# borglab/gtsfm

Measured on NVIDIA H100. Metric: image_pairs_per_sec, higher is better.
Workload: dtype f32

## Files before the change

gtsfm_b200/csrc/gemm_ws.cuh:

```cuda
#pragma once
#include "tma.cuh"

constexpr int GW_MAXP = 16;
constexpr int GW_M = 128, GW_N = 128, GW_K = 64;
constexpr int GW_A_BYTES = GW_M * GW_K * 2;
constexpr int GW_B_BYTES = GW_N * GW_K * 2;
constexpr int GW_STAGE_BYTES = 2 * GW_A_BYTES + 2 * GW_B_BYTES;
constexpr int GW_STAGES = 2;
constexpr int GW_PITCH = GW_N + 8;
constexpr int GW_STG_BYTES = GW_M * GW_PITCH * 4;
constexpr int GW_RB = 8;
constexpr int GW_EW = 4;
constexpr int GW_THREADS = 512;
constexpr size_t GW_SMEM = GW_STAGES * GW_STAGE_BYTES + GW_STG_BYTES + 1024  + 256 ;
constexpr int GW_SEGS = 3;

struct GemmProblem {
  const float* resid;
  float* C;
  __half *Ch[GW_SEGS], *Cl[GW_SEGS];
  const float *cs, *sn;
  int M, N, ldc;
  int vec4;
  int tiles_n;
  int tile_end;
};
struct GemmWsMaps {
  CUtensorMap a1h[GW_MAXP], a1l[GW_MAXP];
  CUtensorMap a2h[GW_MAXP], a2l[GW_MAXP];
  CUtensorMap bh[GW_MAXP], bl[GW_MAXP];
};
struct GemmWsArgs {
  GemmProblem p[GW_MAXP];
  int nprob, tiles;
  int K1, K2;
  int b_per_problem;
  const float* bias;
  int ldr;
  float scale;
  int ldch;
  int head_major;
  int relu;
  int gelu;
  int lo_unscaled;
  int seg_n;
  int rot_mask;
  int* err_flag;
};

static __device__ __noinline__ float gelu_erf(float x) { return 0.5f * x * (1.0f + erff(x * 0.70710678118654752440f)); }

static __global__ void __launch_bounds__(GW_THREADS, 1) k_gemm_ws(const __grid_constant__ GemmWsMaps maps, const __grid_constant__ GemmWsArgs g) {
  extern __shared__ unsigned char gw_raw[];
  const uint32_t raw = tc::smem_u32(gw_raw);
  const uint32_t smem0 = (raw + 1023u) & ~1023u;
  unsigned char* sm = gw_raw + (smem0 - raw);
  float* stg = reinterpret_cast<float*>(sm + GW_STAGES * GW_STAGE_BYTES);
  uint64_t* full = reinterpret_cast<uint64_t*>(sm + GW_STAGES * GW_STAGE_BYTES + GW_STG_BYTES);
  uint64_t* empty = full + GW_STAGES;
  uint64_t* sfull = empty + GW_STAGES;
  uint64_t* sempty = sfull + 1;

  const int t = threadIdx.x, warp = t >> 5, lane = t & 31;
  const int nk = (g.K1 + g.K2) / GW_K;

  if (t == 0) {
    for (int s = 0; s < GW_STAGES; ++s) tc::mbar_init(&full[s], 1), tc::mbar_init(&empty[s], 8);
    tc::mbar_init(sfull, 256);
    tc::mbar_init(sempty, 32 * GW_EW);
    tc::fence_mbar_init();
    tc::tma_prefetch_desc(&maps.bh[0]);
    tc::tma_prefetch_desc(&maps.bl[0]);
  }
  __syncthreads();
  bool ok = true;

  auto decode = [&](int tile, int& z, int& m0, int& n0) {
    z = 0;
    while (z + 1 < g.nprob && tile >= g.p[z].tile_end) ++z;
    const int local = tile - (z ? g.p[z - 1].tile_end : 0);
    const int mt = local / g.p[z].tiles_n;
    n0 = (local - mt * g.p[z].tiles_n) * GW_N;
    m0 = mt * GW_M;
  };

  if (warp >= 12) {
    asm volatile("setmaxnreg.dec.sync.aligned.u32 40;\n" ::: "memory");
    if (warp == 12 && lane == 0) {
      int gk = 0;
      for (int tile = blockIdx.x; tile < g.tiles; tile += gridDim.x) {
        int z, m0, n0;
        decode(tile, z, m0, n0);
        const int zb = g.b_per_problem ? z : 0;
        for (int kc = 0; kc < nk; ++kc, ++gk) {
          const int s = gk % GW_STAGES;
          if (gk >= GW_STAGES) ok = tc::mbar_wait(&empty[s], ((gk / GW_STAGES) - 1) & 1) && ok;
          const int k0 = kc * GW_K;
          const bool seg2 = k0 >= g.K1;
          const CUtensorMap* ah = seg2 ? &maps.a2h[z] : &maps.a1h[z];
          const CUtensorMap* al = seg2 ? &maps.a2l[z] : &maps.a1l[z];
          const int ka = seg2 ? k0 - g.K1 : k0;
          const uint32_t sA = smem0 + s * GW_STAGE_BYTES, sB = sA + 2 * GW_A_BYTES;
          tc::mbar_expect_tx(&full[s], GW_STAGE_BYTES);
          tc::tma_load_2d(sA, ah, &full[s], ka, m0);
          tc::tma_load_2d(sA + GW_A_BYTES, al, &full[s], ka, m0);
          tc::tma_load_2d(sB, &maps.bh[zb], &full[s], k0, n0);
          tc::tma_load_2d(sB + GW_B_BYTES, &maps.bl[zb], &full[s], k0, n0);
        }
      }
    }
  } else if (warp < 8) {
    asm volatile("setmaxnreg.inc.sync.aligned.u32 184;\n" ::: "memory");
    const int wg = warp >> 2;
    const int r0 = wg * 64 + (warp & 3) * 16 + (lane >> 2);
    const int c2 = (lane & 3) * 2;
    int gk = 0, it = 0;
    for (int tile = blockIdx.x; tile < g.tiles; tile += gridDim.x, ++it) {
      float acc0[64], acc1[64];
      for (int kc = 0; kc < nk; ++kc, ++gk) {
        const int s = gk % GW_STAGES;
        ok = tc::mbar_wait(&full[s], (gk / GW_STAGES) & 1) && ok;
        const uint32_t aH = smem0 + s * GW_STAGE_BYTES + wg * (64 * 128), aL = aH + GW_A_BYTES;
        const uint32_t bH = smem0 + s * GW_STAGE_BYTES + 2 * GW_A_BYTES, bL = bH + GW_B_BYTES;
        const uint64_t dAh = tc::wg_desc_sw128(aH), dAl = tc::wg_desc_sw128(aL), dBh = tc::wg_desc_sw128(bH), dBl = tc::wg_desc_sw128(bL);
        tc::wg_fence();
#pragma unroll
        for (int ks = 0; ks < GW_K / 16; ++ks) {
          const uint64_t adv = (uint64_t)(ks * 2);
          const uint32_t first = (kc == 0 && ks == 0) ? 0u : 1u;
          tc::wg_ss_n128(acc0, dAh + adv, dBh + adv, first);
          tc::wg_ss_n128(acc1, dAh + adv, dBl + adv, first);
          tc::wg_ss_n128(acc1, dAl + adv, dBh + adv, 1u);
        }
        tc::wg_commit();
        if (kc > 0) {
          tc::wg_wait<1>();
          if (lane == 0) tc::mbar_arrive(&empty[(gk - 1) % GW_STAGES]);
        }
      }
      tc::wg_wait<0>();
      if (lane == 0) tc::mbar_arrive(&empty[(gk - 1) % GW_STAGES]);

      if (it > 0) ok = tc::mbar_wait(sempty, (it - 1) & 1) && ok;
#pragma unroll
      for (int j = 0; j < 16; ++j)
#pragma unroll
        for (int h = 0; h < 2; ++h) {
          const int i = 4 * j + 2 * h;
          *reinterpret_cast<float2*>(stg + (r0 + 8 * h) * GW_PITCH + 8 * j + c2) =
              make_float2(fmaf(acc1[i], tc::LO_INV, acc0[i]), fmaf(acc1[i + 1], tc::LO_INV, acc0[i + 1]));
        }
      tc::mbar_arrive(sfull);
    }
  } else {
    asm volatile("setmaxnreg.dec.sync.aligned.u32 104;\n" ::: "memory");
    const int ew = warp - 8;
    const int c = 4 * lane;
    const float scale = g.scale;
    const int relu = g.relu, gelu = g.gelu, hm = g.head_major, lo_unscaled = g.lo_unscaled, ldr = g.ldr, ldch = g.ldch;
    int it = 0;
    for (int tile = blockIdx.x; tile < g.tiles; tile += gridDim.x, ++it) {
      int z, m0, n0;
      decode(tile, z, m0, n0);
      const GemmProblem& pb = g.p[z];
      const float* resid = pb.resid;
      float* C = pb.C;
      const int sg = g.seg_n ? n0 / g.seg_n : 0;
      __half *Ch = pb.Ch[sg], *Cl = pb.Cl[sg];
      const bool rot = (g.rot_mask >> sg) & 1;
      const int M = pb.M, ldc = pb.ldc;
      const int n = n0 + c;
      const int ncols = min(4, pb.N - n);
      const bool vec = pb.vec4 && ncols == 4;
      const int rows = min(GW_M, M - m0);
      float b4[4] = {0.f, 0.f, 0.f, 0.f};
      if (g.bias)
#pragma unroll
        for (int e = 0; e < 4; ++e)
          if (e < ncols) b4[e] = __ldg(g.bias + n + e);
      const int ns = n - sg * g.seg_n;
      const size_t hm_col = (size_t)(ns >> 6) * M * 64 + (ns & 63);
      const bool vres = resid && vec;
      const int rp = (ns & 63) >> 1;
      float4 rr[GW_RB];
      auto load_rows = [&](int rb) {
        if (rot) {
#pragma unroll
          for (int i = 0; i < GW_RB; ++i)
            if (rb + GW_EW * i < rows) {
              const size_t o = (size_t)(m0 + rb + GW_EW * i) * 32 + rp;
              const float2 cc = __ldg(reinterpret_cast<const float2*>(pb.cs + o)), ss = __ldg(reinterpret_cast<const float2*>(pb.sn + o));
              rr[i] = make_float4(cc.x, cc.y, ss.x, ss.y);
            }
        } else {
#pragma unroll
          for (int i = 0; i < GW_RB; ++i)
            if (rb + GW_EW * i < rows) rr[i] = *reinterpret_cast<const float4*>(resid + (size_t)(m0 + rb + GW_EW * i) * ldr + n);
        }
      };
      if (vres || rot) load_rows(ew);
      ok = tc::mbar_wait(sfull, it & 1) && ok;
      auto pre = [&](int r, float* v) {
        const float4 a = *reinterpret_cast<const float4*>(stg + r * GW_PITCH + c);
        v[0] = a.x, v[1] = a.y, v[2] = a.z, v[3] = a.w;
#pragma unroll
        for (int e = 0; e < 4; ++e) {
          v[e] = (v[e] + b4[e]) * scale;
          if (relu) v[e] = fmaxf(v[e], 0.f);
          if (gelu) v[e] = gelu_erf(v[e]);
        }
      };
      if (ncols > 0 && vec) {
        for (int rb = ew; rb < rows; rb += GW_EW * GW_RB) {
          if ((vres || rot) && rb != ew) load_rows(rb);
#pragma unroll
          for (int i = 0; i < GW_RB; ++i) {
            const int r = rb + GW_EW * i;
            if (r >= rows) break;
            const int row = m0 + r;
            float v[4];
            pre(r, v);
            if (resid) v[0] += rr[i].x, v[1] += rr[i].y, v[2] += rr[i].z, v[3] += rr[i].w;
            if (rot) {
              const float c0 = rr[i].x, c1 = rr[i].y, s0 = rr[i].z, s1 = rr[i].w;
              const float a0 = __fadd_rn(__fmul_rn(v[0], c0), __fmul_rn(-v[1], s0)), a1 = __fadd_rn(__fmul_rn(v[1], c0), __fmul_rn(v[0], s0));
              const float a2 = __fadd_rn(__fmul_rn(v[2], c1), __fmul_rn(-v[3], s1)), a3 = __fadd_rn(__fmul_rn(v[3], c1), __fmul_rn(v[2], s1));
              v[0] = a0, v[1] = a1, v[2] = a2, v[3] = a3;
            }
            const size_t off = hm ? hm_col + (size_t)row * 64 : (size_t)row * ldc + n;
            if (C) *reinterpret_cast<float4*>(C + off) = make_float4(v[0], v[1], v[2], v[3]);
            if (Ch) {
              const size_t off_s = hm ? off : (size_t)row * ldch + n;
              uint32_t h01, l01, h23, l23;
              if (lo_unscaled) {
                tc::split2_unscaled_clamped(v[0], v[1], h01, l01);
                tc::split2_unscaled_clamped(v[2], v[3], h23, l23);
              } else {
                tc::split2(v[0], v[1], h01, l01);
                tc::split2(v[2], v[3], h23, l23);
              }
              *reinterpret_cast<uint2*>(Ch + off_s) = make_uint2(h01, h23);
              *reinterpret_cast<uint2*>(Cl + off_s) = make_uint2(l01, l23);
            }
          }
        }
      } else if (ncols > 0) {
#pragma unroll 1
        for (int r = ew; r < rows; r += GW_EW) {
          const int row = m0 + r;
          float v[4];
          pre(r, v);
          const size_t off_c = hm ? hm_col + (size_t)row * 64 : (size_t)row * ldc + n;
          const size_t off_s = hm ? hm_col + (size_t)row * 64 : (size_t)row * ldch + n;
#pragma unroll
          for (int e = 0; e < 4; ++e) {
            if (e >= ncols) break;
            if (resid) v[e] += resid[(size_t)row * ldr + n + e];
            if (C) C[off_c + e] = v[e];
            if (Ch) {
              __half hh, ll;
              if (lo_unscaled) tc::split_h_unscaled(v[e], hh, ll);
              else tc::split_h(v[e], hh, ll);
              Ch[off_s + e] = hh;
              Cl[off_s + e] = ll;
            }
          }
        }
      }
      tc::mbar_arrive(sempty);
    }
  }
  if (!ok && g.err_flag) *g.err_flag = 1;
}
```

gtsfm_b200/csrc/linear.cuh:

```cuda
#pragma once
#include "attn_ps.cuh"
#include "common.cuh"
#include "gemm.cuh"
#include "gemm_ws.cuh"

struct TcWeights {
  const float* f;
  const __half* h;
  const __half* l;
  int* err;
  bool use_tc;
  DevBuf* attn_part = nullptr;
  DevBuf* attn_ml = nullptr;
  DevBuf* attn_cnt = nullptr;
  int sm_count = 132;
};

struct Pl {
  __half* hi;
  __half* lo;
};
static inline Pl planes_of(const DevBuf& b, size_t elems) { return {b.as<__half>(), b.as<__half>() + elems}; }

struct LinArgs {
  const float* a1f = nullptr;
  Pl a1p{nullptr, nullptr};
  int lda1 = 0, K1 = 0;
  const float* a2f = nullptr;
  Pl a2p{nullptr, nullptr};
  int lda2 = 0, K2 = 0;
  const float* w = nullptr;
  const float* bf = nullptr;
  Pl bp{nullptr, nullptr};
  int ldb = 0;
  const float* bias = nullptr;
  float scale = 1.f;
  const float* resid = nullptr;
  int ldr = 0;
  float* cf = nullptr;
  int ldc = 0;
  Pl cp{nullptr, nullptr};
  int ldch = 0;
  int head_major = 0;
  bool tc_want_f32 = false;
  int relu = 0;
  int gelu = 0;
  int lo_unscaled = 0;
  int M = 0, N = 0;
  int seg_n = 0;
  float* seg_f[GW_SEGS] = {};
  Pl seg_p[GW_SEGS] = {};
  int rot_mask = 0;
  const float *cs = nullptr, *sn = nullptr;
};

static int run_linear(b2_context* ctx, cudaStream_t st, const TcWeights& tw, const LinArgs* a, int np, const char* site = nullptr) {
  if (np <= 0) return B2_OK;
  if (np > GW_MAXP) return b2_fail(ctx, B2_ERR_ARG, "run_linear: too many problems in one launch");
  const LinArgs& a0 = a[0];
  const int nseg = a0.seg_n > 0 ? a0.N / a0.seg_n : 1;
  if (a0.seg_n > 0 && (a0.seg_n % GW_N || a0.N != nseg * a0.seg_n || nseg > GW_SEGS || !a0.head_major || a0.resid || a0.tc_want_f32 ||
                       (a0.rot_mask && (!a0.cs || !a0.sn))))
    return b2_fail(ctx, B2_ERR_ARG, "run_linear: column segments need N = seg_n x (<= 3), seg_n % 128 == 0, head-major planes, "
                                    "no residual or fp32 output, and a rotary table when rotary is on");
  if (!tw.use_tc) {
    if (a0.rot_mask) return b2_fail(ctx, B2_ERR_ARG, "run_linear: the rotary epilogue exists on the wgmma path only");
    for (int i = 0; i < np; ++i) {
      const LinArgs& x = a[i];
      if (x.M <= 0 || x.N <= 0) continue;
      if (x.gelu) return b2_fail(ctx, B2_ERR_ARG, "run_linear: the GELU epilogue exists on the wgmma path only");
      if (x.K1 % GB_K || x.K2 % GB_K || x.lda1 % 4 || x.lda2 % 4 || x.ldb % 4)
        return b2_fail(ctx, B2_ERR_ARG, "run_linear: the SIMT GEMM needs K1, K2 multiples of 16 and lda1, lda2, ldb multiples of 4");
    }
    for (int i = 0; i < np; ++i) {
      const LinArgs& x = a[i];
      if (x.M <= 0 || x.N <= 0) continue;
      for (int s = 0; s < nseg; ++s) {
        const int c0 = s * x.seg_n;
        GemmArgs g{};
        g.A1 = x.a1f, g.lda1 = x.lda1, g.K1 = x.K1, g.A2 = x.a2f, g.lda2 = x.lda2, g.K2 = x.K2;
        g.B = (x.w ? x.w : x.bf) + (size_t)c0 * x.ldb, g.ldb = x.ldb, g.C = x.seg_n ? x.seg_f[s] : x.cf, g.ldc = x.ldc, g.M = x.M;
        g.N = x.seg_n ? x.seg_n : x.N;
        g.bias = x.bias ? x.bias + c0 : nullptr, g.resid = x.resid, g.ldr = x.ldr, g.scale = x.scale, g.head_major = x.head_major;
        g.relu = x.relu;
        int rc = launch_gemm(ctx, st, g);
        if (rc) return rc;
      }
    }
    return B2_OK;
  }
  if (a0.K1 % GW_K || a0.K2 % GW_K) return b2_fail(ctx, B2_ERR_ARG, "run_linear: the wgmma GEMM needs K1 and K2 multiples of 64");
  if (!tma_encoder()) return b2_fail(ctx, B2_ERR_CUDA, "cuTensorMapEncodeTiled is not available (driver too old?)");
  const bool per_b = a0.w == nullptr;
  static thread_local GemmWsMaps maps;
  GemmWsArgs q{};
  double work = 0.0;
  bool ok = true;
  int nz = 0, tiles = 0;
  for (int i = 0; i < np; ++i) {
    const LinArgs& x = a[i];
    if (x.M <= 0 || x.N <= 0) continue;
    ok = ok && tma_map_2d(&maps.a1h[nz], x.a1p.hi, x.M, x.K1, x.lda1, GW_M) && tma_map_2d(&maps.a1l[nz], x.a1p.lo, x.M, x.K1, x.lda1, GW_M);
    if (x.K2 > 0)
      ok = ok && tma_map_2d(&maps.a2h[nz], x.a2p.hi, x.M, x.K2, x.lda2, GW_M) && tma_map_2d(&maps.a2l[nz], x.a2p.lo, x.M, x.K2, x.lda2, GW_M);
    if (per_b || nz == 0) {
      const __half *bh, *bl;
      if (x.w) {
        const size_t off = (size_t)(x.w - tw.f);
        bh = tw.h + off, bl = tw.l + off;
      } else {
        bh = x.bp.hi, bl = x.bp.lo;
      }
      ok = ok && tma_map_2d(&maps.bh[nz], bh, x.N, x.K1 + x.K2, x.ldb, GW_N) && tma_map_2d(&maps.bl[nz], bl, x.N, x.K1 + x.K2, x.ldb, GW_N);
    }
    GemmProblem& pr = q.p[nz];
    pr.resid = x.resid, pr.C = x.tc_want_f32 ? x.cf : nullptr, pr.M = x.M, pr.N = x.N, pr.ldc = x.ldc;
    for (int s = 0; s < GW_SEGS; ++s) {
      const Pl p = x.seg_n ? (s < nseg ? x.seg_p[s] : Pl{nullptr, nullptr}) : (s == 0 ? x.cp : Pl{nullptr, nullptr});
      pr.Ch[s] = p.hi, pr.Cl[s] = p.lo;
    }
    pr.cs = x.cs, pr.sn = x.sn;
    {
      auto al16 = [](const void* q) { return (reinterpret_cast<uintptr_t>(q) & 15) == 0; };
      auto al8 = [](const void* q) { return (reinterpret_cast<uintptr_t>(q) & 7) == 0; };
      const bool hm = x.head_major != 0;
      bool v = al16(pr.resid) && (x.ldr % 4 == 0 || !pr.resid) && al16(pr.C) && (hm || x.ldc % 4 == 0 || !pr.C);
      v = v && (hm || x.ldch % 4 == 0 || !pr.Ch[0]);
      for (int s = 0; s < GW_SEGS; ++s) v = v && al8(pr.Ch[s]) && al8(pr.Cl[s]);
      v = v && al8(pr.cs) && al8(pr.sn);
      pr.vec4 = v ? 1 : 0;
      if (x.seg_n && !v) return b2_fail(ctx, B2_ERR_ARG, "run_linear: column segments need 8-byte aligned planes and rotary tables");
    }
    pr.tiles_n = cdiv(x.N, GW_N);
    tiles += cdiv(x.M, GW_M) * pr.tiles_n;
    pr.tile_end = tiles;
    work += 2.0 * x.M * x.N * (x.K1 + x.K2);
    ++nz;
  }
  if (nz == 0) return B2_OK;
  if (!ok) return b2_fail(ctx, B2_ERR_CUDA, "cuTensorMapEncodeTiled failed");
  q.nprob = nz, q.tiles = tiles, q.K1 = a0.K1, q.K2 = a0.K2, q.b_per_problem = per_b ? 1 : 0;
  q.bias = a0.bias, q.ldr = a0.ldr, q.scale = a0.scale, q.ldch = a0.ldch;
  q.head_major = a0.head_major, q.relu = a0.relu, q.gelu = a0.gelu, q.lo_unscaled = a0.lo_unscaled, q.err_flag = tw.err;
  q.seg_n = a0.seg_n, q.rot_mask = a0.rot_mask;
  const std::string name = site ? std::string("k_gemm_ws/") + site : std::string("k_gemm_ws");
  b2_prof_work(ctx, name.c_str(), work);
  B2_LAUNCH_NAMED(ctx, name.c_str(), k_gemm_ws, tiles < tw.sm_count ? tiles : tw.sm_count, GW_THREADS, GW_SMEM, st, maps, q);
  B2_CHECK_LAUNCH(ctx);
  return B2_OK;
}

struct FlashPlanes {
  Pl q, k, v, o;
  int nq, nk;
  int heads, ldo;
};
static int run_flash_planes(b2_context* ctx, cudaStream_t st, const TcWeights& tw, const FlashPlanes* jobs, int np, float scale,
                            bool fp16_single = false) {
  if (np <= 0) return B2_OK;
  if (np > AP_MAXP) return b2_fail(ctx, B2_ERR_ARG, "run_flash: too many problems in one launch");
  if (!tma_encoder() || !tw.attn_part) return b2_fail(ctx, B2_ERR_CUDA, "wgmma attention needs cuTensorMapEncodeTiled and its scratch buffers");
  static thread_local AttnPsMaps tmaps;
  AttnPsArgs pa{};
  bool okm = true;
  int items = 0, nz = 0, W = 0, tmax = 0;
  double work = 0.0;
  for (int i = 0; i < np; ++i) {
    const FlashPlanes& j = jobs[i];
    if (j.nq <= 0 || j.nk <= 0) continue;
    AttnPsProblem& p = pa.p[nz];
    p.Qh = j.q.hi, p.Ql = j.q.lo, p.Oh = j.o.hi, p.Ol = j.o.lo, p.Nq = j.nq, p.Nk = j.nk, p.ldo = j.ldo;
    p.qt = cdiv(j.nq, 2 * AW_Q), p.tiles = cdiv(j.nk, AW_KV);
    p.item0 = items;
    items += p.qt * j.heads;
    W += p.qt * j.heads * p.tiles;
    p.w_end = W;
    tmax = p.tiles > tmax ? p.tiles : tmax;
    const uint64_t rows = (uint64_t)j.heads * j.nk;
    okm = okm && tma_map_2d(&tmaps.kh[nz], j.k.hi, rows, 64, 64, AW_KV) && tma_map_2d(&tmaps.kl[nz], j.k.lo, rows, 64, 64, AW_KV);
    okm = okm && tma_map_2d(&tmaps.vh[nz], j.v.hi, rows, 64, 64, AW_KV) && tma_map_2d(&tmaps.vl[nz], j.v.lo, rows, 64, 64, AW_KV);
    work += j.heads * 2.0 * 2.0 * 64 * (double)j.nq * j.nk;
    ++nz;
  }
  if (nz == 0) return B2_OK;
  if (!okm) return b2_fail(ctx, B2_ERR_CUDA, "cuTensorMapEncodeTiled failed (attention)");
  pa.nprob = nz, pa.W = W;
  int ncta = W < tw.sm_count ? W : tw.sm_count;
  pa.quota = cdiv(W, ncta);
  ncta = cdiv(W, pa.quota);
  pa.max_splits = cdiv(tmax, pa.quota) + 1;
  B2_CUDA(ctx, tw.attn_part->ensure((size_t)items * pa.max_splits * 256 * 64 * 4));
  B2_CUDA(ctx, tw.attn_ml->ensure((size_t)items * pa.max_splits * 256 * 2 * 4));
  {
    DevBuf& cnt = *tw.attn_cnt;
    const size_t need = (size_t)items * 2 * sizeof(int);
    if (cnt.cap < need) {
      B2_CUDA(ctx, cnt.ensure(need * 4));
      B2_CUDA(ctx, cudaMemsetAsync(cnt.p, 0, cnt.cap, st));
    }
    pa.arrivals = cnt.as<int>();
  }
  pa.Opart = tw.attn_part->as<float>(), pa.ml = tw.attn_ml->as<float>();
  pa.scale = scale, pa.err_flag = tw.err;
  b2_prof_work(ctx, "k_flash_ps", work);
  if (fp16_single) B2_LAUNCH(ctx, k_flash_ps<true>, ncta, AS_THREADS, AS_SMEM, st, tmaps, pa);
  else B2_LAUNCH(ctx, k_flash_ps<false>, ncta, AS_THREADS, AS_SMEM, st, tmaps, pa);
  B2_CHECK_LAUNCH(ctx);
  return B2_OK;
}

struct FlashJob {
  const DevBuf *q, *k, *v, *o;
  int nq, nk;
  int capq, capk;
};
static int run_flash(b2_context* ctx, cudaStream_t st, const TcWeights& tw, const FlashJob* jobs, int np, float scale, bool fp16_single = false) {
  if (np <= 0) return B2_OK;
  if (np > AP_MAXP) return b2_fail(ctx, B2_ERR_ARG, "run_flash: too many problems in one launch");
  if (!tw.use_tc) {
    for (int i = 0; i < np; ++i) {
      const FlashJob& j = jobs[i];
      int rc = launch_flash(ctx, st, j.q->as<float>(), j.k->as<float>(), j.v->as<float>(), j.o->as<float>(), j.nq, j.nk, scale);
      if (rc) return rc;
    }
    return B2_OK;
  }
  FlashPlanes fp[AP_MAXP];
  for (int i = 0; i < np; ++i) {
    const FlashJob& j = jobs[i];
    fp[i] = {planes_of(*j.q, (size_t)j.capq * 256), planes_of(*j.k, (size_t)j.capk * 256), planes_of(*j.v, (size_t)j.capk * 256),
             planes_of(*j.o, (size_t)j.capq * 256), j.nq, j.nk, 4, 256};
  }
  return run_flash_planes(ctx, st, tw, fp, np, scale, fp16_single);
}
```

gtsfm_b200/csrc/tma.cuh:

```cuda
#pragma once
#include <cuda.h>
#include <cuda_fp16.h>

#include "common.cuh"
#include "tc.cuh"

namespace tc {
__device__ __forceinline__ void mbar_expect_tx(uint64_t* bar, uint32_t bytes) {
  asm volatile("mbarrier.arrive.expect_tx.shared::cta.b64 _, [%0], %1;" ::"r"(smem_u32(bar)), "r"(bytes) : "memory");
}
__device__ __forceinline__ void tma_load_2d(uint32_t dst_smem, const CUtensorMap* map, uint64_t* bar, int x, int y) {
  asm volatile(
      "cp.async.bulk.tensor.2d.shared::cluster.global.tile.mbarrier::complete_tx::bytes [%0], [%1, {%3, %4}], [%2];"
      ::"r"(dst_smem), "l"(reinterpret_cast<uint64_t>(map)), "r"(smem_u32(bar)), "r"(x), "r"(y)
      : "memory");
}
__device__ __forceinline__ void tma_prefetch_desc(const CUtensorMap* map) {
  asm volatile("prefetch.tensormap [%0];" ::"l"(reinterpret_cast<uint64_t>(map)) : "memory");
}
}

typedef CUresult (*PFN_encodeTiled)(CUtensorMap*, CUtensorMapDataType, cuuint32_t, void*, const cuuint64_t*, const cuuint64_t*,
                                    const cuuint32_t*, const cuuint32_t*, CUtensorMapInterleave, CUtensorMapSwizzle,
                                    CUtensorMapL2promotion, CUtensorMapFloatOOBfill);

static inline PFN_encodeTiled tma_encoder() {
  static PFN_encodeTiled fn = nullptr;
  if (!fn) {
    void* p = nullptr;
    cudaDriverEntryPointQueryResult q;
    if (cudaGetDriverEntryPoint("cuTensorMapEncodeTiled", &p, cudaEnableDefault, &q) == cudaSuccess && q == cudaDriverEntryPointSuccess)
      fn = reinterpret_cast<PFN_encodeTiled>(p);
  }
  return fn;
}

static inline bool tma_map_2d(CUtensorMap* out, const __half* base, uint64_t rows, uint64_t cols, uint64_t ld, uint32_t box_rows) {
  PFN_encodeTiled enc = tma_encoder();
  if (!enc || !base) return false;
  cuuint64_t dims[2] = {cols, rows};
  cuuint64_t strides[1] = {ld * sizeof(__half)};
  cuuint32_t box[2] = {64, box_rows};
  cuuint32_t estr[2] = {1, 1};
  return enc(out, CU_TENSOR_MAP_DATA_TYPE_FLOAT16, 2, const_cast<__half*>(base), dims, strides, box, estr, CU_TENSOR_MAP_INTERLEAVE_NONE,
             CU_TENSOR_MAP_SWIZZLE_128B, CU_TENSOR_MAP_L2_PROMOTION_L2_256B, CU_TENSOR_MAP_FLOAT_OOB_FILL_NONE) == CUDA_SUCCESS;
}

static __global__ void k_split_f32(const float* __restrict__ x, size_t n, __half* __restrict__ hi, __half* __restrict__ lo) {
  size_t i = (size_t)blockIdx.x * blockDim.x + threadIdx.x;
  if (i >= n) return;
  __half h, l;
  tc::split_h(x[i], h, l);
  hi[i] = h;
  lo[i] = l;
}
```

Baseline: 130.9.

## Route GEMM epilogue stores through swizzled smem and TMA bulk tensor stores

Result: faster. 132.5 (median of 6 runs) (+1.2%).

```diff
diff --git a/gtsfm_b200/csrc/gemm_ws.cuh b/gtsfm_b200/csrc/gemm_ws.cuh
--- a/gtsfm_b200/csrc/gemm_ws.cuh
+++ b/gtsfm_b200/csrc/gemm_ws.cuh
@@ -7,8 +7,8 @@
 constexpr int GW_B_BYTES = GW_N * GW_K * 2;
 constexpr int GW_STAGE_BYTES = 2 * GW_A_BYTES + 2 * GW_B_BYTES;
 constexpr int GW_STAGES = 2;
-constexpr int GW_PITCH = GW_N + 8;
-constexpr int GW_STG_BYTES = GW_M * GW_PITCH * 4;
+constexpr int GW_BLK = GW_M * 128;
+constexpr int GW_STG_BYTES = 4 * GW_BLK;
 constexpr int GW_RB = 8;
 constexpr int GW_EW = 4;
 constexpr int GW_THREADS = 512;
@@ -29,6 +29,8 @@
   CUtensorMap a1h[GW_MAXP], a1l[GW_MAXP];
   CUtensorMap a2h[GW_MAXP], a2l[GW_MAXP];
   CUtensorMap bh[GW_MAXP], bl[GW_MAXP];
+  CUtensorMap c[GW_MAXP];
+  CUtensorMap ch[GW_MAXP][GW_SEGS], cl[GW_MAXP][GW_SEGS];
 };
 struct GemmWsArgs {
   GemmProblem p[GW_MAXP];
@@ -67,7 +69,7 @@
   if (t == 0) {
     for (int s = 0; s < GW_STAGES; ++s) tc::mbar_init(&full[s], 1), tc::mbar_init(&empty[s], 8);
     tc::mbar_init(sfull, 256);
-    tc::mbar_init(sempty, 32 * GW_EW);
+    tc::mbar_init(sempty, 1);
     tc::fence_mbar_init();
     tc::tma_prefetch_desc(&maps.bh[0]);
     tc::tma_prefetch_desc(&maps.bl[0]);
@@ -147,7 +149,8 @@
 #pragma unroll
         for (int h = 0; h < 2; ++h) {
           const int i = 4 * j + 2 * h;
-          *reinterpret_cast<float2*>(stg + (r0 + 8 * h) * GW_PITCH + 8 * j + c2) =
+          const int off = (j >> 2) * GW_BLK + (r0 + 8 * h) * 128 + (((2 * (j & 3) + (c2 >> 2)) ^ (lane >> 2)) << 4) + (c2 & 3) * 4;
+          *reinterpret_cast<float2*>(reinterpret_cast<unsigned char*>(stg) + off) =
               make_float2(fmaf(acc1[i], tc::LO_INV, acc0[i]), fmaf(acc1[i + 1], tc::LO_INV, acc0[i + 1]));
         }
       tc::mbar_arrive(sfull);
@@ -156,8 +159,14 @@
     asm volatile("setmaxnreg.dec.sync.aligned.u32 104;\n" ::: "memory");
     const int ew = warp - 8;
     const int c = 4 * lane;
+    const bool leader = t == 256;
     const float scale = g.scale;
     const int relu = g.relu, gelu = g.gelu, hm = g.head_major, lo_unscaled = g.lo_unscaled, ldr = g.ldr, ldch = g.ldch;
+    unsigned char* stgb = reinterpret_cast<unsigned char*>(stg);
+    const uint32_t stg_s = tc::smem_u32(stg);
+    const int o32_0 = (lane >> 3) * GW_BLK + (((lane & 7) ^ ew) << 4), o32_1 = o32_0 ^ (4 << 4);
+    const int oh_0 = 2 * (lane >> 4) * GW_BLK + ((((lane & 15) >> 1) ^ ew) << 4) + (lane & 1) * 8, oh_1 = oh_0 ^ (4 << 4);
+    auto epi_sync = [] { asm volatile("bar.sync 1, 128;" ::: "memory"); };
     int it = 0;
     for (int tile = blockIdx.x; tile < g.tiles; tile += gridDim.x, ++it) {
       int z, m0, n0;
@@ -168,10 +177,10 @@
       const int sg = g.seg_n ? n0 / g.seg_n : 0;
       __half *Ch = pb.Ch[sg], *Cl = pb.Cl[sg];
       const bool rot = (g.rot_mask >> sg) & 1;
-      const int M = pb.M, ldc = pb.ldc;
+      const int M = pb.M, N = pb.N, ldc = pb.ldc;
       const int n = n0 + c;
-      const int ncols = min(4, pb.N - n);
-      const bool vec = pb.vec4 && ncols == 4;
+      const int ncols = min(4, N - n);
+      const bool fast = pb.vec4 != 0;
       const int rows = min(GW_M, M - m0);
       float b4[4] = {0.f, 0.f, 0.f, 0.f};
       if (g.bias)
@@ -179,8 +188,7 @@
         for (int e = 0; e < 4; ++e)
           if (e < ncols) b4[e] = __ldg(g.bias + n + e);
       const int ns = n - sg * g.seg_n;
-      const size_t hm_col = (size_t)(ns >> 6) * M * 64 + (ns & 63);
-      const bool vres = resid && vec;
+      const bool vres = resid && fast && ncols > 0;
       const int rp = (ns & 63) >> 1;
       float4 rr[GW_RB];
       auto load_rows = [&](int rb) {
@@ -200,9 +208,8 @@
       };
       if (vres || rot) load_rows(ew);
       ok = tc::mbar_wait(sfull, it & 1) && ok;
-      auto pre = [&](int r, float* v) {
-        const float4 a = *reinterpret_cast<const float4*>(stg + r * GW_PITCH + c);
-        v[0] = a.x, v[1] = a.y, v[2] = a.z, v[3] = a.w;
+      auto ld_row = [&](int r, int p) { return *reinterpret_cast<const float4*>(stgb + r * 128 + (p ? o32_1 : o32_0)); };
+      auto fin = [&](float* v) {
 #pragma unroll
         for (int e = 0; e < 4; ++e) {
           v[e] = (v[e] + b4[e]) * scale;
@@ -210,46 +217,113 @@
           if (gelu) v[e] = gelu_erf(v[e]);
         }
       };
-      if (ncols > 0 && vec) {
-        for (int rb = ew; rb < rows; rb += GW_EW * GW_RB) {
-          if ((vres || rot) && rb != ew) load_rows(rb);
-#pragma unroll
-          for (int i = 0; i < GW_RB; ++i) {
-            const int r = rb + GW_EW * i;
-            if (r >= rows) break;
-            const int row = m0 + r;
-            float v[4];
-            pre(r, v);
-            if (resid) v[0] += rr[i].x, v[1] += rr[i].y, v[2] += rr[i].z, v[3] += rr[i].w;
-            if (rot) {
-              const float c0 = rr[i].x, c1 = rr[i].y, s0 = rr[i].z, s1 = rr[i].w;
-              const float a0 = __fadd_rn(__fmul_rn(v[0], c0), __fmul_rn(-v[1], s0)), a1 = __fadd_rn(__fmul_rn(v[1], c0), __fmul_rn(v[0], s0));
-              const float a2 = __fadd_rn(__fmul_rn(v[2], c1), __fmul_rn(-v[3], s1)), a3 = __fadd_rn(__fmul_rn(v[3], c1), __fmul_rn(v[2], s1));
-              v[0] = a0, v[1] = a1, v[2] = a2, v[3] = a3;
-            }
-            const size_t off = hm ? hm_col + (size_t)row * 64 : (size_t)row * ldc + n;
-            if (C) *reinterpret_cast<float4*>(C + off) = make_float4(v[0], v[1], v[2], v[3]);
-            if (Ch) {
-              const size_t off_s = hm ? off : (size_t)row * ldch + n;
-              uint32_t h01, l01, h23, l23;
-              if (lo_unscaled) {
-                tc::split2_unscaled_clamped(v[0], v[1], h01, l01);
-                tc::split2_unscaled_clamped(v[2], v[3], h23, l23);
-              } else {
-                tc::split2(v[0], v[1], h01, l01);
-                tc::split2(v[2], v[3], h23, l23);
+      auto put_planes = [&](int r, int p, const float* v, bool sync = true) {
+        uint32_t h01, l01, h23, l23;
+        if (lo_unscaled) {
+          tc::split2_unscaled_clamped(v[0], v[1], h01, l01);
+          tc::split2_unscaled_clamped(v[2], v[3], h23, l23);
+        } else {
+          tc::split2(v[0], v[1], h01, l01);
+          tc::split2(v[2], v[3], h23, l23);
+        }
+        unsigned char* q = stgb + r * 128 + (p ? oh_1 : oh_0);
+        if (sync) __syncwarp();
+        *reinterpret_cast<uint2*>(q) = make_uint2(h01, h23);
+        *reinterpret_cast<uint2*>(q + GW_BLK) = make_uint2(l01, l23);
+      };
+      auto store_half = [&](int hf, bool f32) {
+        const int y = m0 + 64 * hf;
+        const uint32_t src = stg_s + hf * 64 * 128;
+        if (f32) {
+#pragma unroll 1
+          for (int b = 0; b < 4; ++b) {
+            const int col = n0 + 32 * b;
+            if (col < N) tc::tma_store_3d(&maps.c[z], src + b * GW_BLK, hm ? (col & 63) : col, y, hm ? col >> 6 : 0);
+          }
+        } else {
+#pragma unroll 1
+          for (int k = 0; k < 2; ++k) {
+            const int col = n0 + 64 * k;
+            if (col >= N) break;
+            const int x = hm ? 0 : col, h = hm ? (col - sg * g.seg_n) >> 6 : 0;
+            tc::tma_store_3d(&maps.ch[z][sg], src + 2 * k * GW_BLK, x, y, h);
+            tc::tma_store_3d(&maps.cl[z][sg], src + (2 * k + 1) * GW_BLK, x, y, h);
+          }
+        }
+        tc::bulk_commit();
+      };
+      if (fast) {
+        const bool direct_planes = Ch && !C;
+        for (int hf = 0; hf < 2 && 64 * hf < rows; ++hf) {
+          for (int rb = 64 * hf + ew; rb < 64 * (hf + 1) && rb < rows; rb += GW_EW * GW_RB) {
+            if ((vres || rot) && rb != ew) load_rows(rb);
+            auto post = [&](int i, float* v) {
+              if (vres) v[0] += rr[i].x, v[1] += rr[i].y, v[2] += rr[i].z, v[3] += rr[i].w;
+              if (rot) {
+                const float c0 = rr[i].x, c1 = rr[i].y, s0 = rr[i].z, s1 = rr[i].w;
+                const float a0 = __fadd_rn(__fmul_rn(v[0], c0), __fmul_rn(-v[1], s0)), a1 = __fadd_rn(__fmul_rn(v[1], c0), __fmul_rn(v[0], s0));
+                const float a2 = __fadd_rn(__fmul_rn(v[2], c1), __fmul_rn(-v[3], s1)), a3 = __fadd_rn(__fmul_rn(v[3], c1), __fmul_rn(v[2], s1));
+                v[0] = a0, v[1] = a1, v[2] = a2, v[3] = a3;
               }
-              *reinterpret_cast<uint2*>(Ch + off_s) = make_uint2(h01, h23);
-              *reinterpret_cast<uint2*>(Cl + off_s) = make_uint2(l01, l23);
-            }
+            };
+            if (direct_planes && !gelu) {
+#pragma unroll
+              for (int i0 = 0; i0 < GW_RB; i0 += 4) {
+                float4 ab[4];
+#pragma unroll
+                for (int i = 0; i < 4; ++i)
+                  if (rb + GW_EW * (i0 + i) < rows) ab[i] = ld_row(rb + GW_EW * (i0 + i), i & 1);
+                __syncwarp();
+#pragma unroll
+                for (int i = 0; i < 4; ++i) {
+                  const int r = rb + GW_EW * (i0 + i);
+                  if (r >= rows) break;
+                  float v[4] = {ab[i].x, ab[i].y, ab[i].z, ab[i].w};
+                  fin(v);
+                  post(i0 + i, v);
+                  put_planes(r, i & 1, v, false);
+                }
+              }
+              continue;
+            }
+            float4 a = ld_row(rb, 0);
+#pragma unroll
+            for (int i = 0; i < GW_RB; ++i) {
+              const int r = rb + GW_EW * i;
+              if (r >= rows) break;
+              float v[4] = {a.x, a.y, a.z, a.w};
+              if (i + 1 < GW_RB && r + GW_EW < rows) a = ld_row(r + GW_EW, (i + 1) & 1);
+              fin(v);
+              post(i, v);
+              if (direct_planes) put_planes(r, i & 1, v);
+              else *reinterpret_cast<float4*>(stgb + r * 128 + ((i & 1) ? o32_1 : o32_0)) = make_float4(v[0], v[1], v[2], v[3]);
+            }
+          }
+          tc::fence_proxy_async();
+          epi_sync();
+          if (leader) store_half(hf, C != nullptr);
+          if (C && Ch) {
+            if (leader) tc::bulk_wait_read<0>();
+            epi_sync();
+#pragma unroll 1
+            for (int r = 64 * hf + ew; r < 64 * (hf + 1) && r < rows; r += GW_EW) {
+              const float4 a = ld_row(r, (r >> 2) & 1);
+              const float v[4] = {a.x, a.y, a.z, a.w};
+              put_planes(r, (r >> 2) & 1, v);
+            }
+            tc::fence_proxy_async();
+            epi_sync();
+            if (leader) store_half(hf, false);
           }
         }
       } else if (ncols > 0) {
+        const size_t hm_col = (size_t)(ns >> 6) * M * 64 + (ns & 63);
 #pragma unroll 1
         for (int r = ew; r < rows; r += GW_EW) {
           const int row = m0 + r;
-          float v[4];
-          pre(r, v);
+          const float4 a = ld_row(r, (r >> 2) & 1);
+          float v[4] = {a.x, a.y, a.z, a.w};
+          fin(v);
           const size_t off_c = hm ? hm_col + (size_t)row * 64 : (size_t)row * ldc + n;
           const size_t off_s = hm ? hm_col + (size_t)row * 64 : (size_t)row * ldch + n;
 #pragma unroll
@@ -267,7 +341,11 @@
           }
         }
       }
-      tc::mbar_arrive(sempty);
+      epi_sync();
+      if (leader) {
+        tc::bulk_wait_read<0>();
+        tc::mbar_arrive(sempty);
+      }
     }
   }
   if (!ok && g.err_flag) *g.err_flag = 1;
diff --git a/gtsfm_b200/csrc/linear.cuh b/gtsfm_b200/csrc/linear.cuh
--- a/gtsfm_b200/csrc/linear.cuh
+++ b/gtsfm_b200/csrc/linear.cuh
@@ -124,12 +124,21 @@
       auto al16 = [](const void* q) { return (reinterpret_cast<uintptr_t>(q) & 15) == 0; };
       auto al8 = [](const void* q) { return (reinterpret_cast<uintptr_t>(q) & 7) == 0; };
       const bool hm = x.head_major != 0;
-      bool v = al16(pr.resid) && (x.ldr % 4 == 0 || !pr.resid) && al16(pr.C) && (hm || x.ldc % 4 == 0 || !pr.C);
-      v = v && (hm || x.ldch % 4 == 0 || !pr.Ch[0]);
-      for (int s = 0; s < GW_SEGS; ++s) v = v && al8(pr.Ch[s]) && al8(pr.Cl[s]);
+      bool v = al16(pr.resid) && (!pr.resid || (x.ldr % 4 == 0 && x.N % 4 == 0)) && al16(pr.C) && (!pr.C || hm || (x.ldc % 4 == 0 && x.N % 4 == 0));
+      v = v && (!pr.Ch[0] || hm || (x.ldch % 8 == 0 && x.N % 8 == 0)) && (!hm || x.N % 64 == 0);
+      for (int s = 0; s < GW_SEGS; ++s) v = v && al16(pr.Ch[s]) && al16(pr.Cl[s]);
       v = v && al8(pr.cs) && al8(pr.sn);
       pr.vec4 = v ? 1 : 0;
-      if (x.seg_n && !v) return b2_fail(ctx, B2_ERR_ARG, "run_linear: column segments need 8-byte aligned planes and rotary tables");
+      if (x.seg_n && !v) return b2_fail(ctx, B2_ERR_ARG, "run_linear: column segments need 16-byte aligned planes and 8-byte aligned rotary tables");
+      if (v) {
+        const uint64_t M = x.M, N = x.N, heads = (x.seg_n ? x.seg_n : x.N) / 64;
+        auto map = [&](CUtensorMap* m, const void* base, bool f32, uint64_t ld) {
+          return hm ? tma_map_store(m, base, f32, 64, M, heads, 64, M * 64) : tma_map_store(m, base, f32, N, M, 1, ld, M * ld);
+        };
+        if (pr.C) ok = ok && map(&maps.c[nz], pr.C, true, x.ldc);
+        for (int s = 0; s < GW_SEGS; ++s)
+          if (pr.Ch[s]) ok = ok && map(&maps.ch[nz][s], pr.Ch[s], false, x.ldch) && map(&maps.cl[nz][s], pr.Cl[s], false, x.ldch);
+      }
     }
     pr.tiles_n = cdiv(x.N, GW_N);
     tiles += cdiv(x.M, GW_M) * pr.tiles_n;
diff --git a/gtsfm_b200/csrc/tma.cuh b/gtsfm_b200/csrc/tma.cuh
--- a/gtsfm_b200/csrc/tma.cuh
+++ b/gtsfm_b200/csrc/tma.cuh
@@ -17,6 +17,16 @@
 }
 __device__ __forceinline__ void tma_prefetch_desc(const CUtensorMap* map) {
   asm volatile("prefetch.tensormap [%0];" ::"l"(reinterpret_cast<uint64_t>(map)) : "memory");
+}
+__device__ __forceinline__ void tma_store_3d(const CUtensorMap* map, uint32_t src_smem, int x, int y, int z) {
+  asm volatile("cp.async.bulk.tensor.3d.global.shared::cta.bulk_group [%0, {%2, %3, %4}], [%1];"
+               ::"l"(reinterpret_cast<uint64_t>(map)), "r"(src_smem), "r"(x), "r"(y), "r"(z)
+               : "memory");
+}
+__device__ __forceinline__ void bulk_commit() { asm volatile("cp.async.bulk.commit_group;" ::: "memory"); }
+template <int N>
+__device__ __forceinline__ void bulk_wait_read() {
+  asm volatile("cp.async.bulk.wait_group.read %0;" ::"n"(N) : "memory");
 }
 }
 
@@ -46,6 +56,20 @@
              CU_TENSOR_MAP_SWIZZLE_128B, CU_TENSOR_MAP_L2_PROMOTION_L2_256B, CU_TENSOR_MAP_FLOAT_OOB_FILL_NONE) == CUDA_SUCCESS;
 }
 
+static inline bool tma_map_store(CUtensorMap* out, const void* base, bool f32, uint64_t inner, uint64_t rows, uint64_t outer,
+                                 uint64_t ld, uint64_t outer_ld) {
+  PFN_encodeTiled enc = tma_encoder();
+  if (!enc || !base) return false;
+  const uint64_t es = f32 ? 4 : 2;
+  cuuint64_t dims[3] = {inner, rows, outer};
+  cuuint64_t strides[2] = {ld * es, outer_ld * es};
+  cuuint32_t box[3] = {(cuuint32_t)(128 / es), 64, 1};
+  cuuint32_t estr[3] = {1, 1, 1};
+  return enc(out, f32 ? CU_TENSOR_MAP_DATA_TYPE_FLOAT32 : CU_TENSOR_MAP_DATA_TYPE_FLOAT16, 3, const_cast<void*>(base), dims, strides, box,
+             estr, CU_TENSOR_MAP_INTERLEAVE_NONE, CU_TENSOR_MAP_SWIZZLE_128B, CU_TENSOR_MAP_L2_PROMOTION_NONE,
+             CU_TENSOR_MAP_FLOAT_OOB_FILL_NONE) == CUDA_SUCCESS;
+}
+
 static __global__ void k_split_f32(const float* __restrict__ x, size_t n, __half* __restrict__ hi, __half* __restrict__ lo) {
   size_t i = (size_t)blockIdx.x * blockDim.x + threadIdx.x;
   if (i >= n) return;
```
